# dallison/subspace

Hardware: AMD Instinct MI355X
Metric: GiB/s CRC32 over batched payloads (device-resident); % of HBM3E read peak (higher is better)
Workload: dtype u8

## Files before the change

### subspace_amd/csrc/capi.hip

```cpp
#include <hip/hip_runtime.h>

#include <algorithm>
#include <cstdarg>
#include <cstdio>
#include <cstring>
#include <mutex>
#include <vector>

#include "../../include/subspace_crc.h"
#include "crc_device.h"
#include "crc_math.h"
#include "ctx.h"

namespace subspace_amd {

template <int WG, bool SLOT, bool PROBE>
__global__ void crc32_uniform4k_kernel(const uint8_t*, u64, u64, const u32*, const u32*, u32, u32, u32*, int, u32*,
                                       SlotArgs);

struct TileDesc;
struct TileDesc8;
__global__ void crc32_ragged_count_desc_kernel(const u64*, u32, const u64*, u32, u64, u32, u32, u64*, u32*, u32*,
                                               u64*, u32*, u64, TileDesc8*, u32*, FaultRef);
__global__ void crc32_ragged_count_desc16_kernel(const u64*, u32, const u64*, u32, u64, u32, u32, u64*, u32*, u32*,
                                                 u64*, u32*, u64, TileDesc*, u32*, FaultRef);
__global__ void crc32_ragged_count_scan_kernel(const u64*, u32, const u64*, u32, u64, u32, u32, u64*, u32*, u32*,
                                               u64*, u32*, u32*, FaultRef);
__global__ void tile_segment_scan_kernel(const u32*, u32, u32, u32, const u64*, u64, u32*, u32*);
__global__ void segment_prefix_kernel(u32*, u64, u32, u32, const u64*, u64, u64*, u32*, FaultRef);
__global__ void crc32_ragged_desc_kernel(const u64*, u32, const u64*, u32, const u64*, u64, u64, TileDesc*, u32*,
                                         u64*, u64, u32*, FaultRef);
template <int WG>
__global__ void crc32_ragged_kernel(const uint8_t*, const u64*, u32, const u64*, u32, const u64*, u64,
                                    const TileDesc*, const u32*, const u32*, const u32*, HeadSeeds, u32*, u32*, u32,
                                    u64*, u64, u32*, FaultRef);
__global__ void crc32_ragged_final_kernel(const u64*, const u64*, u32, const u64*, u32, u64, const u32*, const u32*,
                                          u32, u32, u32*, const u32*, u32, u32*, u64*, u64, u32*, FaultRef);
__global__ void crc32_slot_finish_kernel(const u64*, uint8_t*, u64, const u64*, u64, u64, u64, int, int, u32,
                                         const u32*, const u32*, const u32*, u32*, u32*, u32*);
__global__ void slot_payload_offsets_kernel(u64, u64, u64, u64*, const u64*, u64, u64*);
__global__ void uniform_offsets_kernel(u64 stride, u64 length, u64 count, u64* offsets, u64* lengths);
template <int WG>
__global__ void crc32_long_kernel(const uint8_t*, u64, u32, u32, const u32*, const u32*, u32, u32, u32*, u32);
__global__ void crc32_long_final_kernel(const u32*, const u32*, u32, u32, u32, u32, u32*, u64*, u64, u32*);
template <int WG, bool SLOT, bool PROBE, int G>
__global__ void crc32_small_kernel(const u32*, const u32*, SmallArgs);

}

using namespace subspace_amd;

namespace {

thread_local char g_err[512] = "";

int fail(int code, const char* fmt, ...) {
  va_list ap;
  va_start(ap, fmt);
  vsnprintf(g_err, sizeof(g_err), fmt, ap);
  va_end(ap);
  return code;
}
int hip_fail(hipError_t e, const char* what) {
  return fail(SUBSPACE_CRC_EHIP, "%s: %s", what, hipGetErrorString(e));
}
#define HIP_TRY(call)                                   \
  do {                                                  \
    hipError_t e_ = (call);                             \
    if (e_ != hipSuccess) return hip_fail(e_, #call);   \
  } while (0)

constexpr int kRaggedWG = 512;

struct HostRegion {
  uintptr_t host;
  uint64_t bytes;
  uintptr_t dev;
};
std::mutex g_regions_mu;
std::vector<HostRegion> g_regions;

uintptr_t host_alias(uintptr_t p, uint64_t n) {
  for (const auto& r : g_regions)
    if (p >= r.host && p - r.host <= r.bytes && n <= r.bytes - (p - r.host)) return r.dev + (p - r.host);
  return 0;
}
#ifndef SUBSPACE_FINAL_BLOCKS_PER_CU
#define SUBSPACE_FINAL_BLOCKS_PER_CU 2
#endif
constexpr size_t kTileDescBytes = 16;
constexpr u64 ceil_div(u64 a, u64 b) { return (a + b - 1) / b; }

// ... 118 lines not shown
    c->scan_b_words = ceil_div(tile_geom(c, c->desc_capacity).nseg, kScanTile);
    HIP_TRY(hipMalloc(&c->d_scan_state, (1 + c->scan_a_words + c->scan_b_words) * sizeof(u64)));
    HIP_TRY(hipMemset(c->d_scan_state, 0, (1 + c->scan_a_words + c->scan_b_words) * sizeof(u64)));
    HIP_TRY(hipDeviceSynchronize());
    c->scan_dirty = false;
  }
  if (!c->d_overflow) {
    HIP_TRY(hipMalloc(&c->d_overflow, 16));
    HIP_TRY(hipMemset(c->d_overflow, 0, 16));
    HIP_TRY(hipDeviceSynchronize());
  }
  return SUBSPACE_CRC_OK;
}

int scan_state_clean(subspace_crc_ctx* c, hipStream_t st) {
  if (c->scan_dirty) {
    HIP_TRY(hipMemsetAsync(c->d_scan_state, 0, (1 + c->scan_a_words + c->scan_b_words) * sizeof(u64), st));
    c->scan_dirty = false;
  }
  return SUBSPACE_CRC_OK;
}

u64 clamp_capacity(const subspace_crc_ctx* c, u64 cap, u64 count) {
  const u64 lim = std::min<u64>(c->mem_tiles + count + 1, (1ull << 32) - (1ull << 20));
  return std::min(cap, lim);
}

FaultRef new_call_fault(subspace_crc_ctx* c) {
  if (++c->call_gen == 0) c->call_gen = 1;
  return FaultRef{c->d_fault, c->call_gen};
}

int combine_tiles(subspace_crc_ctx* c, const TileGeom& g, const u64* total_ptr, u64 tiles, FaultRef fr,
                  hipStream_t st) {
  const dim3 grid((unsigned)ceil_div(g.nkmax, 64), (unsigned)g.nwb);
  tile_segment_scan_kernel<<<grid, 256, 0, st>>>(c->d_tilecrc, (u32)g.nw, (u32)g.nkmax, (u32)g.nwb, total_ptr, tiles,
                                                  c->d_local, c->d_segx);
  HIP_TRY(hipGetLastError());
  u32* tickets = reinterpret_cast<u32*>(c->d_scan_state);
  segment_prefix_kernel<<<(unsigned)ceil_div(g.nseg, kScanTile), 256, 0, st>>>(
      c->d_segx, g.nseg, (u32)g.nw, (u32)g.nwb, total_ptr, tiles, c->d_scan_state + 1 + c->scan_a_words, tickets + 1,
      fr);
  HIP_TRY(hipGetLastError());
  return SUBSPACE_CRC_OK;
}

int grid_for(subspace_crc_ctx* c, u64 work_units, int waves_per_block) {
  const u64 waves = work_units ? work_units : 1;
  u64 blocks = (waves + waves_per_block - 1) / waves_per_block;
  if (blocks > (u64)c->num_cus) blocks = c->num_cus;
  return (int)(blocks ? blocks : 1);
}

int ragged_run(subspace_crc_ctx* c, const uint8_t* base, u64 cap, const u64* offsets, u32 ostride, const u64* lengths,
               u32 lstride, u64 count, u32 init, u32 final_xor, u32* out, hipStream_t st, u64 arena) {
  int rc = use_workspace(c, st);
  if (rc) return rc;
  cap = clamp_capacity(c, cap, count);
  rc = ensure_ragged_ws(c, count, cap);
  if (rc) return rc;
  const TileGeom g = tile_geom(c, cap);
  const u64 n1 = count + 1;
  rc = scan_state_clean(c, st);
  if (rc) return rc;
  c->scan_dirty = true;
  const FaultRef fr = new_call_fault(c);
  u32* tickets = reinterpret_cast<u32*>(c->d_scan_state);
  const bool fused = c->fused_prep && arena != 0 && arena <= (1ull << kDesc8StartBits) && cap / count <= 64;
  const bool fused16 = c->fused_prep && arena == 0 && cap / count <= 64;
  if (fused) {
    crc32_ragged_count_desc_kernel<<<(unsigned)ceil_div(n1, kCountTile), 1024, 0, st>>>(
        offsets, ostride, lengths, lstride, count, init, final_xor, c->d_tbase, out, c->zero_word, c->d_scan_state + 1,
        reinterpret_cast<u32*>(c->d_scan_state), cap, reinterpret_cast<TileDesc8*>(c->d_desc), c->d_overflow, fr);
    c->zero_word = nullptr;
    HIP_TRY(hipGetLastError());
  } else if (fused16) {
    crc32_ragged_count_desc16_kernel<<<(unsigned)ceil_div(n1, kCountTile), 1024, 0, st>>>(
        offsets, ostride, lengths, lstride, count, init, final_xor, c->d_tbase, out, c->zero_word, c->d_scan_state + 1,
        reinterpret_cast<u32*>(c->d_scan_state), cap, reinterpret_cast<TileDesc*>(c->d_desc), c->d_overflow, fr);
    c->zero_word = nullptr;
    HIP_TRY(hipGetLastError());
  } else {
    crc32_ragged_count_scan_kernel<<<(unsigned)ceil_div(n1, kCountTile), 256, 0, st>>>(
        offsets, ostride, lengths, lstride, count, init, final_xor, c->d_tbase, out, c->zero_word, c->d_scan_state + 1,
        reinterpret_cast<u32*>(c->d_scan_state), c->d_overflow + 1, fr);
    c->zero_word = nullptr;
    HIP_TRY(hipGetLastError());
    const u64 dx = ceil_div(count, 256), waves_x = ceil_div(count, 64);
    const u64 dy = std::max<u64>(1, std::min<u64>({4096, ceil_div(8192, waves_x), cap / count}));
    crc32_ragged_desc_kernel<<<dim3((unsigned)dx, (unsigned)dy), 256, 0, st>>>(
        offsets, ostride, lengths, lstride, c->d_tbase, count, cap, reinterpret_cast<TileDesc*>(c->d_desc),
        c->d_overflow, c->d_scan_state + 1, ceil_div(n1, kCountTile), tickets, fr);
    HIP_TRY(hipGetLastError());
  }
  const int blocks = c->num_cus;
  HeadSeeds seeds;
  seeds.v[0] = init;
  for (int r = 1; r < 16; r++) seeds.v[r] = apply(c->zinv1, seeds.v[r - 1]);
  crc32_ragged_kernel<kRaggedWG><<<blocks, kRaggedWG, ragged_lds_bytes(), st>>>(
      base, offsets, ostride, lengths, lstride, c->d_tbase, count, reinterpret_cast<const TileDesc*>(c->d_desc),
      c->d_overflow, c->d_tab, c->d_rops, seeds, out, c->d_tilecrc, (u32)g.nwb, c->d_scan_state + 1,
      ceil_div(n1, kCountTile), tickets, fr);
  HIP_TRY(hipGetLastError());
  rc = combine_tiles(c, g, c->d_tbase + count, cap, fr, st);
  if (rc) return rc;
  const u64 fb = SUBSPACE_FINAL_BLOCKS_PER_CU ? std::min<u64>(ceil_div(count, 1024), (u64)SUBSPACE_FINAL_BLOCKS_PER_CU * c->num_cus)
                                              : ceil_div(count, 1024);
  crc32_ragged_final_kernel<<<(unsigned)fb, 1024, 0, st>>>(
      c->d_tbase, offsets, ostride, lengths, lstride, count, c->d_local, c->d_segx, (u32)g.nw, (u32)g.nwb,
      c->d_overflow, c->d_rops, final_xor, out, c->d_scan_state + 1 + c->scan_a_words, ceil_div(g.nseg, kScanTile),
      tickets + 1, fr);
  HIP_TRY(hipGetLastError());
  c->scan_dirty = false;
  return SUBSPACE_CRC_OK;
}

bool small_fits(u64 max_len, bool aligned16) { return max_len <= (aligned16 ? kSmallMaxExt : kSmallMaxExt - 15); }

u32 small_lanes(u64 max_ext) {
  if (max_ext == 0) return 32;
  u32 g = 1;
  while (g < 32 && 128ull * g < max_ext) g <<= 1;
  return g;
}

struct SmallSlot {
  const u64* prefixes;
  u32 pstride;
  u64 pdelta;
  u64 max_len;
  u32 mode;
  int32_t checksum_size, metadata_size;
  u32 *status, *crc_out, *error_count;
};
int small_run(subspace_crc_ctx* c, const uint8_t* base, const u64* offsets, u32 ostride, const u64* lengths,
              u32 lstride, u64 count, u32 init, u32 final_xor, u32* out, hipStream_t st,
              const SmallSlot* slot = nullptr, u32 g = 32, u64 ustride = 0, u64 ulen = 0) {
  SmallArgs a{};
  a.ustride = ustride;
  a.ulen = ulen;
  a.base = base;
  a.offsets = offsets;
  a.ostride = ostride;
  a.lengths = lengths;
  a.lstride = lstride;
  a.count = count;
  a.init = init;
  a.final_xor = final_xor;
  a.out = out;
  a.rops = c->d_rops;
  a.pow2 = c->d_pow2;
  a.probe = c->dev.probe;
  const bool probe = c->dev.probe && c->dev.small_slot;
  if (probe) g = 32;
  const u64 tiles = ceil_div(count, 64ull / g);
  const u64 per_wave = slot && g == 32 ? kRp2MaxTilesPerWave : kSmallRingTiles;
// ... 33 lines not shown
#undef SMALL_CASE
    }
  }
  HIP_TRY(hipGetLastError());
  return SUBSPACE_CRC_OK;
}

bool small_slot_fused(int32_t checksum_size, int32_t metadata_size) {
  return (u32)checksum_size <= kSlotFusedMaxMeta && (u32)metadata_size <= kSlotFusedMaxMeta;
}

int ensure_slot_ws(subspace_crc_ctx* c, u64 count) {
  if (count <= c->s_capacity) return SUBSPACE_CRC_OK;
  (void)hipFree(c->d_crc0);
  (void)hipFree(c->d_soff);
  (void)hipFree(c->d_slen);
  c->d_crc0 = nullptr;
  c->d_soff = nullptr;
  c->d_slen = nullptr;
  c->s_capacity = 0;
  HIP_TRY(hipMalloc(&c->d_crc0, count * sizeof(u32)));
  HIP_TRY(hipMalloc(&c->d_soff, count * sizeof(u64)));
  HIP_TRY(hipMalloc(&c->d_slen, count * sizeof(u64)));
  c->s_capacity = count;
  return SUBSPACE_CRC_OK;
}

int check_slot_args(int32_t checksum_size, int32_t metadata_size, uint32_t mode) {
  if (mode != SUBSPACE_CRC_SLOT_CALCULATE && mode != SUBSPACE_CRC_SLOT_VERIFY)
    return fail(SUBSPACE_CRC_EINVAL, "unknown slot mode %u", mode);
  if (checksum_size < 4) return fail(SUBSPACE_CRC_EINVAL, "checksum_size %d < 4", checksum_size);
  if (metadata_size < 0) return fail(SUBSPACE_CRC_EINVAL, "metadata_size %d < 0", metadata_size);
  return SUBSPACE_CRC_OK;
}

void want_zeroed(subspace_crc_ctx* c, u32* err) { c->zero_word = err; }
bool was_zeroed(subspace_crc_ctx* c, u32* err) {
  const bool z = err && c->zero_word == nullptr;
  c->zero_word = nullptr;
  return z;
}

int slot_finish(subspace_crc_ctx* c, const u64* slots, uint8_t* buf, u64 stride, const u64* sizes, u64 usize,
                u64 count, u64 max_len, int32_t cs, int32_t ms, u32 mode, u32* status, u32* err, hipStream_t st,
                u32* crc_out = nullptr, bool err_zeroed = false) {
  if (err && !err_zeroed) HIP_TRY(hipMemsetAsync(err, 0, sizeof(u32), st));
  crc32_slot_finish_kernel<<<(unsigned)((count + 255) / 256), 256, 0, st>>>(
      slots, buf, stride, sizes, usize, count, max_len, cs, ms, mode, c->d_crc0, c->d_tab, c->d_pow2, status, err,
      crc_out);
  HIP_TRY(hipGetLastError());
  return SUBSPACE_CRC_OK;
}

}

extern "C" {

int subspace_crc_version(void) { return 100; }

const char* subspace_crc_last_error(void) { return g_err; }

int subspace_crc_ctx_create(int device, subspace_crc_ctx** out) {
  return subspace_crc_ctx_create_poly(device, SUBSPACE_CRC_POLY_IEEE, out);
}

int subspace_crc_ctx_create_poly(int device, uint32_t poly, subspace_crc_ctx** out) {
  g_err[0] = 0;
  if (!out) return fail(SUBSPACE_CRC_EINVAL, "out is null");
  *out = nullptr;
  if (!(poly & 0x80000000u)) return fail(SUBSPACE_CRC_EINVAL, "polynomial 0x%08x has no x^0 term", poly);
  int ndev = 0;
  if (hipGetDeviceCount(&ndev) != hipSuccess || ndev == 0)
    return fail(SUBSPACE_CRC_ENODEV, "no HIP device available");
  if (device < 0 || device >= ndev) return fail(SUBSPACE_CRC_EINVAL, "device %d out of range [0,%d)", device, ndev);
  hipDeviceProp_t prop;
  HIP_TRY(hipGetDeviceProperties(&prop, device));
  if (std::strncmp(prop.gcnArchName, "gfx950", 6) != 0)
    return fail(SUBSPACE_CRC_ENODEV, "device %d is %s, this library is built for gfx950", device, prop.gcnArchName);
  HIP_TRY(hipSetDevice(device));

  auto* c = new subspace_crc_ctx();
  c->layout_bytes = (uint32_t)sizeof(subspace_crc_ctx);
  c->device = device;
  c->num_cus = prop.multiProcessorCount;
  c->mem_tiles = (u64)prop.totalGlobalMem / 8192;
  c->poly = poly;
  c->host_tab = make_tables(poly);
  c->zinv1 = inverse(z_one(c->host_tab));

  std::vector<u32> tab(1024), pow2(64 * 128, 0u), laneops(kSmallLaneOpSlots * 128, 0u), rops(kRagOpWords, 0u);
  for (int k = 0; k < 4; k++)
    for (int b = 0; b < 256; b++) tab[k * 256 + b] = c->host_tab.t[k][b];

  {
    Mat32 z = z_one(c->host_tab);
    for (int k = 0; k < 64; k++, z = mul(z, z)) nibble_tables(z, &pow2[(size_t)k * 128]);
  }

  for (int sl = 0; sl < 32; sl++) {
    u32 nt[128];
    nibble_tables(z_bytes(c->host_tab, 128ull * sl), nt);
    for (int k = 0; k < 8; k++)
      for (int n = 0; n < 16; n++) laneops[((size_t)k * 16 + n) * 32 + sl] = nt[k * 16 + n];
  }
  std::copy(laneops.begin(), laneops.begin() + kLaneOpWords, rops.begin());
  nibble_tables(z_bytes(c->host_tab, 4096), &laneops[128 * kUniSlotOpZ4096]);
// ... 206 lines not shown
        c->d_scan_state + 1 + c->scan_a_words, ceil_div(g.nseg, kScanTile), reinterpret_cast<u32*>(c->d_scan_state) + 1);
    HIP_TRY(hipGetLastError());
    c->scan_dirty = false;
    return SUBSPACE_CRC_OK;
  }
  const bool aligned = (stride % 16) == 0 && ((uintptr_t)dev_base % 16) == 0;
  if (small_fits(length, aligned) && c->small_path && count > 1)
    return small_run(c, static_cast<const uint8_t*>(dev_base), nullptr, 0, nullptr, 0, count, init, final_xor,
                     dev_out, st, nullptr, small_lanes(length + (aligned ? 0 : 15)), stride, length);
  int rc = use_workspace(c, st);
  if (rc) return rc;
  if (count > c->u_capacity) {
    (void)hipFree(c->d_uoff);
    (void)hipFree(c->d_ulen);
    c->d_uoff = c->d_ulen = nullptr;
    c->u_capacity = 0;
    HIP_TRY(hipMalloc(&c->d_uoff, count * sizeof(u64)));
    HIP_TRY(hipMalloc(&c->d_ulen, count * sizeof(u64)));
    c->u_capacity = count;
  }
  uniform_offsets_kernel<<<(unsigned)((count + 255) / 256), 256, 0, st>>>(stride, length, count, c->d_uoff,
                                                                           c->d_ulen);
  HIP_TRY(hipGetLastError());
  const u64 arena = stride * (count - 1) + length;
  return subspace_crc32_batch(c, dev_base, arena, c->d_uoff, c->d_ulen, count, init, flags, dev_out, stream);
}

int subspace_crc32_slots(subspace_crc_ctx* c, const subspace_crc_slot* dev_slots, uint64_t count,
                         uint64_t max_message_size, int32_t checksum_size, int32_t metadata_size, uint32_t mode,
                         uint32_t* dev_status, uint32_t* dev_error_count, void* stream) {
  g_err[0] = 0;
  if (!c) return fail(SUBSPACE_CRC_EINVAL, "ctx is null");
  CallScope scope(c);
  int rc = check_slot_args(checksum_size, metadata_size, mode);
  if (rc) return rc;
  hipStream_t st = (hipStream_t)stream;
  if (count == 0) {
    if (dev_error_count) HIP_TRY(hipMemsetAsync(dev_error_count, 0, sizeof(u32), st));
    return SUBSPACE_CRC_OK;
  }
  if (!dev_slots) return fail(SUBSPACE_CRC_EINVAL, "null device pointer");
  if (count >= (1ull << 32)) return fail(SUBSPACE_CRC_EINVAL, "count %llu exceeds 2^32-1", (unsigned long long)count);
  HIP_TRY(hipSetDevice(c->device));
  const u64* rec = reinterpret_cast<const u64*>(dev_slots);
  const bool small = max_message_size <= kSmallMaxExt && c->small_path;
  if (small && small_slot_fused(checksum_size, metadata_size)) {
    const SmallSlot ss{rec, 3, 0, ~0ull, mode, checksum_size, metadata_size, dev_status, nullptr, dev_error_count};
    return small_run(c, nullptr, rec + 1, 3, rec + 2, 3, count, 0u, 0u, nullptr, st, &ss, small_lanes(max_message_size));
  }
  rc = use_workspace(c, st);
  if (rc) return rc;
  rc = ensure_slot_ws(c, count);
  if (rc) return rc;
  want_zeroed(c, dev_error_count);
  if (small) {
    rc = small_run(c, nullptr, rec + 1, 3, rec + 2, 3, count, 0u, 0u, c->d_crc0, st, nullptr,
                   small_lanes(max_message_size));
  } else {
    const u64 cap = count * ((max_message_size + 15 + 8191) / 8192) + 1;
    rc = ragged_run(c, nullptr, cap, rec + 1, 3, rec + 2, 3, count, 0u, 0u, c->d_crc0, st, 0);
  }
  const bool zeroed = was_zeroed(c, dev_error_count);
  if (rc) return rc;
  return slot_finish(c, rec, nullptr, 0, nullptr, 0, count, ~0ull, checksum_size, metadata_size, mode, dev_status,
                     dev_error_count, st, nullptr, zeroed);
}

}

namespace {

int slots_strided_impl(subspace_crc_ctx* c, void* dev_buffer, uint64_t slot_stride, uint64_t count,
                       uint64_t message_size, const uint64_t* dev_message_sizes, int32_t checksum_size,
                       int32_t metadata_size, uint32_t mode, uint32_t* dev_status, uint32_t* dev_error_count,
                       u32* dev_crc_out, hipStream_t st) {
  int rc = check_slot_args(checksum_size, metadata_size, mode);
  if (rc) return rc;
  if (count == 0) {
    if (dev_error_count) HIP_TRY(hipMemsetAsync(dev_error_count, 0, sizeof(u32), st));
    return SUBSPACE_CRC_OK;
  }
  if (!dev_buffer) return fail(SUBSPACE_CRC_EINVAL, "null device pointer");
  if (((uintptr_t)dev_buffer % 8) || (slot_stride % 8))
    return fail(SUBSPACE_CRC_EINVAL, "prefixes must be 8-B aligned (buffer %p, stride %llu)", dev_buffer,
                (unsigned long long)slot_stride);
  if (count >= (1ull << 32)) return fail(SUBSPACE_CRC_EINVAL, "count %llu exceeds 2^32-1", (unsigned long long)count);
  const u64 prefix_size = ((u64)(48 + checksum_size + metadata_size) + 63) & ~63ull;
  if (!dev_message_sizes && slot_stride < prefix_size + message_size && count > 1)
    return fail(SUBSPACE_CRC_EINVAL, "slot_stride %llu < prefix %llu + message %llu",
                (unsigned long long)slot_stride, (unsigned long long)prefix_size, (unsigned long long)message_size);
  if (dev_message_sizes && slot_stride < prefix_size && count > 1)
    return fail(SUBSPACE_CRC_EINVAL, "slot_stride %llu < prefix %llu", (unsigned long long)slot_stride,
                (unsigned long long)prefix_size);
  HIP_TRY(hipSetDevice(c->device));
  auto* buf = static_cast<uint8_t*>(dev_buffer);
  if (!dev_message_sizes && message_size == 4096 && (u32)metadata_size <= kSlotFusedMaxMeta && slot_stride % 16 == 0 &&
      ((uintptr_t)(buf + prefix_size) % 16) == 0 && c->fused_slots) {
    const u64 tiles = (count + 1) / 2;
    const u64 blocks = std::max<u64>(grid_for(c, tiles, 512 / 64), ceil_div(tiles, 8ull * kSlotRingRounds));
    SlotArgs sa{prefix_size, mode, dev_status, dev_crc_out, dev_error_count,
                c->d_slot_counter + kCountWords * (c->slot_counter_next++ % kSlotCounters), c->dev.probe, c->d_fault,
                (u32)checksum_size, (u32)metadata_size};
    if (c->dev.probe && c->dev.uniform)
      HIP_TRY(c->dev.uniform(true, (unsigned)blocks, st, buf + prefix_size, slot_stride, count, c->d_tab, c->d_laneops,
                             0u, 0xFFFFFFFFu, nullptr, nullptr, sa));
    else
      crc32_uniform4k_kernel<512, true, false><<<(unsigned)blocks, 512, uniform_slot_lds_bytes(8), st>>>(
          buf + prefix_size, slot_stride, count, c->d_tab, c->d_laneops, 0u, 0xFFFFFFFFu, nullptr, 0, nullptr, sa);
    HIP_TRY(hipGetLastError());
    return SUBSPACE_CRC_OK;
  }
  rc = use_workspace(c, st);
  if (rc) return rc;
  rc = ensure_slot_ws(c, count);
  if (rc) return rc;
  want_zeroed(c, dev_error_count);
  if (dev_message_sizes) {
    const u64 area = count > 1 ? slot_stride - prefix_size : ~0ull;
    slot_payload_offsets_kernel<<<(unsigned)((count + 255) / 256), 256, 0, st>>>(
        slot_stride, prefix_size, count, c->d_soff, dev_message_sizes, area, c->d_slen);
    HIP_TRY(hipGetLastError());
    const bool aligned = slot_stride % 16 == 0 && ((uintptr_t)(buf + prefix_size) % 16) == 0;
    if (count > 1 && small_fits(slot_stride - prefix_size, aligned) && c->small_path) {
      if (small_slot_fused(checksum_size, metadata_size)) {
        was_zeroed(c, dev_error_count);
        const SmallSlot ss{c->d_soff, 1, prefix_size, slot_stride - prefix_size, mode, checksum_size, metadata_size,
                           dev_status, dev_crc_out, dev_error_count};
        return small_run(c, buf, c->d_soff, 1, dev_message_sizes, 1, count, 0u, 0u, nullptr, st, &ss,
                         small_lanes(slot_stride - prefix_size + (aligned ? 0 : 15)));
      }
      rc = small_run(c, buf, c->d_soff, 1, c->d_slen, 1, count, 0u, 0u, c->d_crc0, st, nullptr,
                     small_lanes(slot_stride - prefix_size + (aligned ? 0 : 15)));
    } else {
      const u64 cap = (slot_stride * count + 15 * count) / 8192 + count + 1;
      rc = ragged_run(c, buf, cap, c->d_soff, 1, c->d_slen, 1, count, 0u, 0u, c->d_crc0, st,
                      slot_stride * count);
    }
  } else {
    rc = subspace_crc32_batch_uniform(c, buf + prefix_size, slot_stride, message_size, count, 0u, 0u, c->d_crc0,
                                      st);
  }
  const bool zeroed = was_zeroed(c, dev_error_count);
  if (rc) return rc;
  const u64 max_len = dev_message_sizes && count > 1 ? slot_stride - prefix_size : ~0ull;
  return slot_finish(c, nullptr, buf, slot_stride, dev_message_sizes, message_size, count, max_len, checksum_size,
                     metadata_size, mode, dev_status, dev_error_count, st, dev_crc_out, zeroed);
}

}

extern "C" {

int subspace_crc32_slots_strided(subspace_crc_ctx* c, void* dev_buffer, uint64_t slot_stride, uint64_t count,
                                 uint64_t message_size, const uint64_t* dev_message_sizes, int32_t checksum_size,
                                 int32_t metadata_size, uint32_t mode, uint32_t* dev_status,
                                 uint32_t* dev_error_count, void* stream) {
  g_err[0] = 0;
  if (!c) return fail(SUBSPACE_CRC_EINVAL, "ctx is null");
  CallScope scope(c);
  return slots_strided_impl(c, dev_buffer, slot_stride, count, message_size, dev_message_sizes, checksum_size,
                            metadata_size, mode, dev_status, dev_error_count, nullptr, (hipStream_t)stream);
}

int subspace_crc_host_register(void* ptr, uint64_t bytes) {
  g_err[0] = 0;
  if (!ptr || !bytes) return fail(SUBSPACE_CRC_EINVAL, "null pointer or zero size");
  HIP_TRY(hipHostRegister(ptr, bytes, hipHostRegisterMapped | hipHostRegisterPortable));
  void* dev = nullptr;
  hipError_t e = hipHostGetDevicePointer(&dev, ptr, 0);
  if (e != hipSuccess) {
    (void)hipHostUnregister(ptr);
    return hip_fail(e, "hipHostGetDevicePointer");
  }
  std::lock_guard<std::mutex> lock(g_regions_mu);
  g_regions.push_back({reinterpret_cast<uintptr_t>(ptr), bytes, reinterpret_cast<uintptr_t>(dev)});
  return SUBSPACE_CRC_OK;
}

int subspace_crc_host_unregister(void* ptr) {
  g_err[0] = 0;
  if (!ptr) return fail(SUBSPACE_CRC_EINVAL, "null pointer");
  {
    std::lock_guard<std::mutex> lock(g_regions_mu);
    for (size_t i = 0; i < g_regions.size(); i++)
      if (g_regions[i].host == reinterpret_cast<uintptr_t>(ptr)) {
        g_regions.erase(g_regions.begin() + (long)i);
        break;
// ... 225 lines not shown
```

### subspace_amd/csrc/crc_combine.hip

```cpp
#include "crc_desc.h"

namespace subspace_amd {

constexpr int kScanThreads = 256;
constexpr int kScanItems = (int)(kScanTile / kScanThreads);
static_assert(kScanTile % kScanThreads == 0, "segment-prefix scan: whole items per thread");
constexpr int kCountItems = (int)(kCountTile / kScanThreads);
static_assert(kCountTile % kScanThreads == 0, "tile-count scan: whole items per thread");
constexpr u64 kFlagAggregate = 1, kFlagInclusive = 2;

struct SumOp {
  using T = u64;
  static __device__ __forceinline__ T identity() { return 0; }
  static __device__ __forceinline__ T op(T a, T b) { return a + b; }
  static __device__ __forceinline__ u64 pack(u64 flag, T v) { return (flag << 62) | v; }
  static __device__ __forceinline__ u64 flag(u64 s) { return s >> 62; }
  static __device__ __forceinline__ T value(u64 s) { return s & ((1ull << 62) - 1); }
};

struct XorOp {
  using T = u32;
  static __device__ __forceinline__ T identity() { return 0; }
  static __device__ __forceinline__ T op(T a, T b) { return a ^ b; }
  static __device__ __forceinline__ u64 pack(u64 flag, T v) { return (flag << 32) | v; }
// ... 116 lines not shown
  __shared__ u64 sx[kCountTile];
  bool stale;
  const u64 tile = scan_ticket(ticket, fault, &stale, true);
  if (stale) return;
  const u64 base = tile * kCountTile;
  const int tid = threadIdx.x;
#pragma unroll
  for (int j = 0; j < kCountItems; j++) {
    const u64 i = base + (u64)(j * kScanThreads + tid);
    u64 nt = 0;
    if (i < count) {
      const u64 so = offsets[i * ostride];
      nt = msg_tiles(so, lengths[i * lstride]);
      out[i] = nt == 0 ? init ^ final_xor : 0u;
      if (nt && ((((so & ~(u64)15) + ((nt - 1) << 13)) >> kDesc8StartBits) | ((nt - 1) >> kDesc8AfterBits)))
        *wide = 1u;
    } else if (i == count && zero_word) {
      *zero_word = 0u;
    }
    sx[j * kScanThreads + tid] = nt;
  }
  __syncthreads();
  u64 x[kCountItems];
#pragma unroll
  for (int j = 0; j < kCountItems; j++) x[j] = sx[tid * kCountItems + j];
  scan_tile_lookback<SumOp, kCountItems>(x, tile, status, fault);
#pragma unroll
  for (int j = 0; j < kCountItems; j++) sx[tid * kCountItems + j] = x[j];
  __syncthreads();
#pragma unroll
  for (int j = 0; j < kCountItems; j++) {
    const u64 i = base + (u64)(j * kScanThreads + tid);
    if (i <= count) tile_base[i] = sx[j * kScanThreads + tid];
  }
}

constexpr int kFusedThreads = 1024;
constexpr int kFusedItems = (int)(kCountTile / kFusedThreads);
static_assert(kCountTile % kFusedThreads == 0, "fused scan: whole items per thread");
template <bool WIDE>
__device__ __forceinline__ void count_desc_body(const u64* __restrict__ offsets, u32 ostride,
                                                const u64* __restrict__ lengths, u32 lstride, u64 count, u32 init,
                                                u32 final_xor, u64* __restrict__ tile_base, u32* __restrict__ out,
                                                u32* __restrict__ zero_word, u64* __restrict__ status,
                                                u32* __restrict__ ticket, u64 capacity, void* __restrict__ desc,
                                                u32* __restrict__ overflow, FaultRef fault) {
  __shared__ u64 sx[kCountTile];
  __shared__ u32 sw[WIDE ? 1 : kFusedThreads / 64][kDesc8WaveWords][64];
  bool stale;
  const u64 tile = scan_ticket(ticket, fault, &stale, true);
  if (stale) return;
  const u64 base = tile * kCountTile;
  const int tid = threadIdx.x;
  if (WIDE && tid == 0) overflow[1] = 1u;
  u64 so[kFusedItems], L[kFusedItems], nt[kFusedItems];
  bool bad = false;
#pragma unroll
  for (int j = 0; j < kFusedItems; j++) {
    const u64 i = base + (u64)(j * kFusedThreads + tid);
    so[j] = L[j] = nt[j] = 0;
    if (i < count) {
      so[j] = offsets[i * ostride];
      L[j] = lengths[i * lstride];
      nt[j] = msg_tiles(so[j], L[j]);
      out[i] = nt[j] == 0 ? init ^ final_xor : 0u;
      if (!WIDE && nt[j] &&
          ((((so[j] & ~(u64)15) + ((nt[j] - 1) << 13)) >> kDesc8StartBits) | ((nt[j] - 1) >> kDesc8AfterBits)))
        bad = true;
    } else if (i == count && zero_word) {
      *zero_word = 0u;
    }
    sx[j * kFusedThreads + tid] = nt[j];
  }
  if (bad) overflow[2] = 1u;
  __syncthreads();
  u64 x[kFusedItems];
#pragma unroll
  for (int j = 0; j < kFusedItems; j++) x[j] = sx[tid * kFusedItems + j];
  scan_tile_lookback<SumOp, kFusedItems, kFusedThreads>(x, tile, status, fault);
#pragma unroll
  for (int j = 0; j < kFusedItems; j++) sx[tid * kFusedItems + j] = x[j];
  __syncthreads();
#pragma unroll
  for (int j = 0; j < kFusedItems; j++) {
    const u64 i = base + (u64)(j * kFusedThreads + tid);
    const u64 tb = sx[j * kFusedThreads + tid];
    if (i <= count) tile_base[i] = tb;
    if (i == count) overflow[0] = tb > capacity ? 1u : 0u;
    if constexpr (WIDE)
      descw_wave(static_cast<TileDesc*>(desc), capacity, tb, nt[j], so[j], L[j]);
    else
      desc8_wave(static_cast<TileDesc8*>(desc), capacity, tb, nt[j], so[j], L[j], 0u, 64u, sw[tid >> 6], true);
  }
}

__global__ __launch_bounds__(kFusedThreads) void crc32_ragged_count_desc_kernel(
    const u64* __restrict__ offsets, u32 ostride, const u64* __restrict__ lengths, u32 lstride, u64 count, u32 init,
    u32 final_xor, u64* __restrict__ tile_base, u32* __restrict__ out, u32* __restrict__ zero_word,
    u64* __restrict__ status, u32* __restrict__ ticket, u64 capacity, TileDesc8* __restrict__ desc8,
    u32* __restrict__ overflow, FaultRef fault) {
  count_desc_body<false>(offsets, ostride, lengths, lstride, count, init, final_xor, tile_base, out, zero_word, status,
                         ticket, capacity, desc8, overflow, fault);
}

__global__ __launch_bounds__(kFusedThreads) void crc32_ragged_count_desc16_kernel(
    const u64* __restrict__ offsets, u32 ostride, const u64* __restrict__ lengths, u32 lstride, u64 count, u32 init,
    u32 final_xor, u64* __restrict__ tile_base, u32* __restrict__ out, u32* __restrict__ zero_word,
// ... 92 lines not shown
```

### subspace_amd/csrc/crc_slots.hip

```cpp
#include "crc_device.h"

namespace subspace_amd {

constexpr int kSlotWG = 256;
constexpr u32 kHasChecksum = 4u;

__device__ __forceinline__ u32 tab_step4(const u32* __restrict__ t, u32 x) {
  return t[768 + (x & 0xFFu)] ^ t[512 + ((x >> 8) & 0xFFu)] ^ t[256 + ((x >> 16) & 0xFFu)] ^ t[x >> 24];
}
__device__ __forceinline__ u32 tab_step1(const u32* __restrict__ t, u32 crc, u32 b) {
  return (crc >> 8) ^ t[(crc ^ b) & 0xFFu];
}

__device__ u32 crc_bytes(const u32* __restrict__ t, u32 crc, const uint8_t* p, u64 n) {
  while (n && ((uintptr_t)p & 3u)) {
    crc = tab_step1(t, crc, *p++);
    n--;
  }
  const u32* q = reinterpret_cast<const u32*>(p);
  for (; n >= 4; n -= 4) crc = tab_step4(t, crc ^ *q++);
  p = reinterpret_cast<const uint8_t*>(q);
  while (n--) crc = tab_step1(t, crc, *p++);
  return crc;
}

__global__ __launch_bounds__(kSlotWG) void crc32_slot_finish_kernel(
    const u64* __restrict__ slots, uint8_t* __restrict__ buf, u64 stride, const u64* __restrict__ sizes, u64 usize,
    u64 count, u64 max_len, int checksum_size, int metadata_size, u32 mode, const u32* __restrict__ crc0,
    const u32* __restrict__ gtab, const u32* __restrict__ gpow2, u32* __restrict__ status,
    u32* __restrict__ error_count, u32* __restrict__ crc_out) {
  __shared__ u32 t[1024];
  constexpr int kPowLds = 16;
  __shared__ u32 pw2[kPowLds * 128];
  for (int i = threadIdx.x; i < 1024; i += kSlotWG) t[i] = gtab[i];
  for (int i = threadIdx.x; i < kPowLds * 128; i += kSlotWG) pw2[i] = gpow2[i];
  __syncthreads();
  const u64 i = (u64)blockIdx.x * kSlotWG + threadIdx.x;
  if (i >= count) return;
  uint8_t* prefix = slots ? reinterpret_cast<uint8_t*>(slots[3 * i]) : buf + i * stride;
  const u64 len = slots ? slots[3 * i + 2] : (sizes ? sizes[i] : usize);
  u32* pw = reinterpret_cast<u32*>(prefix);
  if (len > max_len) {
    if (status) status[i] = 4u;
    return;
  }

  u32 w[12];
#pragma unroll
  for (int k = 1; k < 12; k++) w[k] = pw[k];
  const bool calc = mode == 0u;
  const bool has = (w[8] & kHasChecksum) != 0u;
  if (calc && !has) {
    w[8] |= kHasChecksum;
    pw[8] = w[8];
  }
  if (!calc && !has) {
    if (status) status[i] = 2u;
    return;
  }
  u32 h = 0xFFFFFFFFu;
#pragma unroll
  for (int k = 1; k < 12; k++) h = tab_step4(t, h ^ w[k]);
  if (metadata_size > 0) h = crc_bytes(t, h, prefix + 48 + checksum_size, (u64)metadata_size);
  u32 zh = h;
  {
    u64 n = len;
    for (int k = 0; n; k++, n >>= 1) {
      if (!(n & 1u)) continue;
      const u32* op = k < kPowLds ? pw2 + 128 * k : gpow2 + 128 * k;
      u32 r = 0;
#pragma unroll
      for (int j = 0; j < 8; j++) r ^= op[16 * j + ((zh >> (4 * j)) & 15u)];
      zh = r;
    }
  }
  const u32 crc = ~(zh ^ crc0[i]);
  if (calc) {
    pw[12] = crc;
    if (status) status[i] = 0u;
    if (crc_out) crc_out[i] = crc;
  } else {
    const bool ok = pw[12] == crc;
    if (status) status[i] = ok ? 0u : 1u;
    if (!ok && error_count) atomicAdd(error_count, 1u);
  }
}

__global__ void slot_payload_offsets_kernel(u64 stride, u64 prefix_size, u64 count, u64* __restrict__ offsets,
                                            const u64* __restrict__ sizes, u64 max_len, u64* __restrict__ clamped) {
  const u64 i = (u64)blockIdx.x * blockDim.x + threadIdx.x;
  if (i >= count) return;
  offsets[i] = i * stride + prefix_size;
  const u64 L = sizes[i];
  clamped[i] = L > max_len ? 0 : L;
}

}
```

### subspace_amd/csrc/ctx.h

```cpp
#pragma once
#include <hip/hip_runtime.h>

#include <mutex>

#include "../../include/subspace_crc.h"
#include "crc_device.h"
#include "crc_math.h"

namespace subspace_amd {

struct DevHooks {
  u64* probe = nullptr;
  hipError_t (*uniform)(bool slot, unsigned blocks, hipStream_t st, const uint8_t* base, u64 stride, u64 count,
                        const u32* tab, const u32* ops, u32 init, u32 final_xor, u32* out, u32* zero_word,
                        SlotArgs sa) = nullptr;
  hipError_t (*small_slot)(unsigned blocks, size_t lds, hipStream_t st, const u32* tab, const u32* ops,
                           const SmallArgs& a) = nullptr;
};

constexpr uint32_t kCtxMagic = 0x43524353u;

}

struct subspace_crc_ctx {
// ... 4 lines not shown
  int num_cus = 256;
  subspace_amd::u32* d_tab = nullptr;
  subspace_amd::u32* d_rops = nullptr;
  subspace_amd::u32* d_pow2 = nullptr;
  subspace_amd::u32* d_laneops = nullptr;
  subspace_amd::Tables host_tab;
  subspace_amd::Mat32 zinv1;
  subspace_amd::u64* d_tbase = nullptr;
  subspace_amd::u64 ws_messages = 0;
  uint8_t* d_desc = nullptr;
  subspace_amd::u32* d_tilecrc = nullptr;
  subspace_amd::u32* d_local = nullptr;
  subspace_amd::u32* d_segx = nullptr;
  subspace_amd::u64 desc_capacity = 0;
  subspace_amd::u64* d_scan_state = nullptr;
  subspace_amd::u64 scan_a_words = 0, scan_b_words = 0;
  bool scan_dirty = false;
  subspace_amd::u64 mem_tiles = 0;
  subspace_amd::u32* d_overflow = nullptr;
  bool fused_prep = true;
  int uniform_blocks = 0;
  int uniform_order = 0;
  bool long_path = true;
  subspace_amd::u32* zero_word = nullptr;
  subspace_amd::u64* d_uoff = nullptr;
  subspace_amd::u64* d_ulen = nullptr;
  subspace_amd::u64 u_capacity = 0;
  hipStream_t hcompute = nullptr;
  struct HostStage {
    hipStream_t stream = nullptr;
    hipEvent_t copied = nullptr;
    hipEvent_t done = nullptr;
    uint8_t* dbuf = nullptr;
    subspace_amd::u64* dsizes = nullptr;
    subspace_amd::u32* dres = nullptr;
    subspace_amd::u32* derr = nullptr;
    subspace_amd::u32* hres = nullptr;
    subspace_amd::u32* herr = nullptr;
  } hstage[2];
  subspace_amd::u64 h_bytes = 0, h_slots = 0;
  subspace_crc_slot* l_hrec = nullptr;
  subspace_crc_slot* l_drec = nullptr;
  subspace_amd::u32* l_dstatus = nullptr;
  subspace_amd::u32* l_hstatus = nullptr;
  subspace_amd::u64 l_capacity = 0;
  subspace_amd::u32* d_crc0 = nullptr;
  subspace_amd::u64* d_soff = nullptr;
  subspace_amd::u64* d_slen = nullptr;
  subspace_amd::u64 s_capacity = 0;
  subspace_amd::u64* d_slot_counter = nullptr;
  subspace_amd::u32 slot_counter_next = 0;
  bool fused_slots = true;
  bool small_path = true;
  subspace_amd::DevHooks dev;
  subspace_amd::u32* d_fault = nullptr;
  subspace_amd::u32 call_gen = 0;
  std::recursive_mutex mu;
  int depth = 0;
  hipEvent_t ws_done = nullptr;
  hipStream_t ws_stream = nullptr;
  bool ws_recorded = false;
  bool ws_waited = false;
  hipStream_t ws_call_stream = nullptr;
};
```

### subspace_amd/csrc/devtools.hip

```cpp
#define SUBSPACE_DEV_TU 1
#include "crc_small.hip"
#include "crc_uniform.hip"
#include "ctx.h"

#include <algorithm>
#include <cstring>

namespace subspace_amd {
template __global__ void crc32_small_kernel<512, true, true, 32>(const u32*, const u32*, SmallArgs);
template __global__ void crc32_uniform4k_kernel<512, false, true>(const uint8_t*, u64, u64, const u32*, const u32*, u32,
                                                                  u32, u32*, int, u32*, SlotArgs);
template __global__ void crc32_uniform4k_kernel<512, true, true>(const uint8_t*, u64, u64, const u32*, const u32*, u32,
                                                                 u32, u32*, int, u32*, SlotArgs);
template __global__ void crc32_uniform4k_kernel<512, false, false>(const uint8_t*, u64, u64, const u32*, const u32*,
                                                                   u32, u32, u32*, int, u32*, SlotArgs);
}

using namespace subspace_amd;

namespace {

bool ctx_ok(const subspace_crc_ctx* c) {
  return c && c->magic == kCtxMagic && c->layout_bytes == (uint32_t)sizeof(subspace_crc_ctx);
}
// ... 9 lines not shown
                         SlotArgs sa) {
  if (slot)
    crc32_uniform4k_kernel<512, true, true><<<blocks, 512, uniform_slot_lds_bytes(8), st>>>(
        base, stride, count, tab, ops, init, final_xor, out, 0, zero_word, sa);
  else
    crc32_uniform4k_kernel<512, false, true><<<blocks, 512, uniform_lds_bytes(8), st>>>(
        base, stride, count, tab, ops, init, final_xor, out, 0, zero_word, sa);
  return hipGetLastError();
}

hipError_t small_slot_probe(unsigned blocks, size_t lds, hipStream_t st, const u32* tab, const u32* ops,
                            const SmallArgs& a) {
  crc32_small_kernel<512, true, true, 32><<<blocks, 512, lds, st>>>(tab, ops, a);
  return hipGetLastError();
}

hipError_t set_lds_attributes() {
  static hipError_t e = [] {
    hipError_t r = hipFuncSetAttribute((const void*)crc32_uniform4k_kernel<512, false, true>,
                                       hipFuncAttributeMaxDynamicSharedMemorySize, (int)uniform_lds_bytes(8));
    if (r == hipSuccess)
      r = hipFuncSetAttribute((const void*)crc32_uniform4k_kernel<512, true, true>,
                              hipFuncAttributeMaxDynamicSharedMemorySize, (int)uniform_slot_lds_bytes(8));
    if (r == hipSuccess)
      r = hipFuncSetAttribute((const void*)crc32_uniform4k_kernel<512, false, false>,
                              hipFuncAttributeMaxDynamicSharedMemorySize, (int)uniform_lds_bytes(8));
    if (r == hipSuccess)
      r = hipFuncSetAttribute((const void*)crc32_small_kernel<512, true, true, 32>,
                              hipFuncAttributeMaxDynamicSharedMemorySize, (int)small_lds_bytes() + 16);
    return r;
  }();
  return e;
}

}

extern "C" {

int subspace_crc_testutil_set(subspace_crc_ctx* c, const char* key, int value) {
  if (!ctx_ok(c) || !key) return SUBSPACE_CRC_EINVAL;
  std::lock_guard<std::recursive_mutex> lk(c->mu);
  if (!std::strcmp(key, "stale_ticket")) {
    if (!c->d_scan_state) return SUBSPACE_CRC_EINVAL;
    const u32 v = (u32)value;
    if (hipSetDevice(c->device) != hipSuccess || hipDeviceSynchronize() != hipSuccess ||
        hipMemcpy(c->d_scan_state, &v, sizeof(u32), hipMemcpyHostToDevice) != hipSuccess)
      return SUBSPACE_CRC_EHIP;
    return SUBSPACE_CRC_OK;
  }
  bool* knob = !std::strcmp(key, "long_path")     ? &c->long_path
               : !std::strcmp(key, "fused_slots") ? &c->fused_slots
               : !std::strcmp(key, "fused_prep")  ? &c->fused_prep
               : !std::strcmp(key, "small_path")  ? &c->small_path
                                                  : nullptr;
  if (!knob) return SUBSPACE_CRC_EINVAL;
  *knob = value != 0;
  return SUBSPACE_CRC_OK;
}

int subspace_crc_testutil_tune(subspace_crc_ctx* c, int uniform_wg, int uniform_blocks, int uniform_order) {
  if (!ctx_ok(c) || uniform_wg != 512 || uniform_order < 0 || uniform_order > 3 || uniform_blocks < 0)
    return SUBSPACE_CRC_EINVAL;
  std::lock_guard<std::recursive_mutex> lk(c->mu);
  c->uniform_blocks = uniform_blocks;
  c->uniform_order = uniform_order;
  return SUBSPACE_CRC_OK;
}

int subspace_crc_testutil_probe(subspace_crc_ctx* c, void* dev_words) {
  if (!ctx_ok(c)) return SUBSPACE_CRC_EINVAL;
  std::lock_guard<std::recursive_mutex> lk(c->mu);
  if (dev_words) {
    if (hipSetDevice(c->device) != hipSuccess || set_lds_attributes() != hipSuccess) return SUBSPACE_CRC_EHIP;
    c->dev.uniform = uniform_probe;
    c->dev.small_slot = small_slot_probe;
  }
  c->dev.probe = static_cast<u64*>(dev_words);
  return SUBSPACE_CRC_OK;
}

uint64_t subspace_crc_testutil_probe_waves(subspace_crc_ctx* c, uint64_t count) {
  if (!ctx_ok(c)) return 0;
  const u64 tiles = (count + 1) / 2;
  return std::max<u64>((u64)blocks_for(c, tiles), (tiles + 8ull * kRp2MaxTilesPerWave - 1) / (8ull * kRp2MaxTilesPerWave)) * 8u;
}

int subspace_crc_testutil_uniform_alias(subspace_crc_ctx* c, const void* dev_base, uint64_t count, uint32_t* dev_out,
                                        void* stream) {
  if (!ctx_ok(c) || !dev_base || !dev_out || count == 0 || ((uintptr_t)dev_base % 16)) return SUBSPACE_CRC_EINVAL;
  std::lock_guard<std::recursive_mutex> lk(c->mu);
  if (hipSetDevice(c->device) != hipSuccess || set_lds_attributes() != hipSuccess) return SUBSPACE_CRC_EHIP;
  const u64 tiles = (count + 1) / 2;
  crc32_uniform4k_kernel<512, false, false><<<blocks_for(c, tiles), 512, uniform_lds_bytes(8), (hipStream_t)stream>>>(
      static_cast<const uint8_t*>(dev_base), 0, count, c->d_tab, c->d_laneops, 0u, 0u, dev_out, 0, nullptr, SlotArgs{});
  return hipGetLastError() == hipSuccess ? SUBSPACE_CRC_OK : SUBSPACE_CRC_EHIP;
}

int subspace_crc_testutil_fault_words(subspace_crc_ctx* c, uint32_t* host_words, void* stream) {
  if (!ctx_ok(c) || !host_words) return SUBSPACE_CRC_EINVAL;
  std::lock_guard<std::recursive_mutex> lk(c->mu);
  if (hipSetDevice(c->device) != hipSuccess ||
      hipMemcpyAsync(host_words, c->d_fault, 2 * sizeof(u32), hipMemcpyDeviceToHost, (hipStream_t)stream) != hipSuccess ||
      hipStreamSynchronize((hipStream_t)stream) != hipSuccess)
    return SUBSPACE_CRC_EHIP;
  return SUBSPACE_CRC_OK;
}

// ... 4 lines not shown
```

Baseline: 5642.

## Fuse ragged tile combine and final pass into slot finish kernel

For slot-based ragged CRC with bounded message sizes, the tile-combine scan, segment prefix and ragged final kernels are skipped. A new slot_combine_finish kernel XORs each message's tile CRCs directly, undoes the padding shift with nibble inverse operators held in LDS, and writes the checksum or verifies it in the same pass. This removes several kernel launches and their intermediate global traffic, at the cost of a serial per-message loop over tiles that is limited to a small tile count.

```diff
diff --git a/subspace_amd/csrc/capi.hip b/subspace_amd/csrc/capi.hip
--- a/subspace_amd/csrc/capi.hip
+++ b/subspace_amd/csrc/capi.hip
@@ -38,6 +38,11 @@
                                           u32, u32, u32*, const u32*, u32, u32*, u64*, u64, u32*, FaultRef);
 __global__ void crc32_slot_finish_kernel(const u64*, uint8_t*, u64, const u64*, u64, u64, u64, int, int, u32,
                                          const u32*, const u32*, const u32*, u32*, u32*, u32*);
+template <bool LIST>
+__global__ void crc32_slot_combine_finish_kernel(const u64*, uint8_t*, u64, const u64*, u64, u64, int, int, u32,
+                                                 const u64*, const u64*, u32, const u64*, u32, const u32*, u32, u32,
+                                                 u32*, const u32*, const u32*, const u32*, const u32*, u32*, u32*,
+                                                 u32*, FaultRef);
 __global__ void slot_payload_offsets_kernel(u64, u64, u64, u64*, const u64*, u64, u64*);
 __global__ void uniform_offsets_kernel(u64 stride, u64 length, u64 count, u64* offsets, u64* lengths);
 template <int WG>
@@ -262,8 +267,14 @@
   return (int)(blocks ? blocks : 1);
 }
 
+struct RaggedTiles {
+  TileGeom g;
+  FaultRef fr;
+};
+
 int ragged_run(subspace_crc_ctx* c, const uint8_t* base, u64 cap, const u64* offsets, u32 ostride, const u64* lengths,
-               u32 lstride, u64 count, u32 init, u32 final_xor, u32* out, hipStream_t st, u64 arena) {
+               u32 lstride, u64 count, u32 init, u32 final_xor, u32* out, hipStream_t st, u64 arena,
+               RaggedTiles* tiles_only = nullptr) {
   int rc = use_workspace(c, st);
   if (rc) return rc;
   cap = clamp_capacity(c, cap, count);
@@ -312,6 +323,11 @@
       c->d_overflow, c->d_tab, c->d_rops, seeds, out, c->d_tilecrc, (u32)g.nwb, c->d_scan_state + 1,
       ceil_div(n1, kCountTile), tickets, fr);
   HIP_TRY(hipGetLastError());
+  if (tiles_only) {
+    tiles_only->g = g;
+    tiles_only->fr = fr;
+    return SUBSPACE_CRC_OK;
+  }
   rc = combine_tiles(c, g, c->d_tbase + count, cap, fr, st);
   if (rc) return rc;
   const u64 fb = SUBSPACE_FINAL_BLOCKS_PER_CU ? std::min<u64>(ceil_div(count, 1024), (u64)SUBSPACE_FINAL_BLOCKS_PER_CU * c->num_cus)
@@ -451,6 +467,38 @@
   return SUBSPACE_CRC_OK;
 }
 
+constexpr u64 kSlotCombineMaxTiles = 8;
+constexpr int kSlotCombineWG = 256;
+bool slot_combine_fits(const subspace_crc_ctx* c, u64 bound) {
+  return c->slot_combine && bound <= kSlotCombineMaxTiles * 8192 - 15;
+}
+
+int ragged_slot_combine(subspace_crc_ctx* c, const uint8_t* base, u64 cap, const u64* offsets, u32 ostride,
+                        const u64* lengths, u32 lstride, u64 arena, const u64* slots, uint8_t* buf, u64 stride,
+                        const u64* sizes, u64 count, u64 max_len, int32_t cs, int32_t ms, u32 mode, u32* status,
+                        u32* err, u32* crc_out, hipStream_t st) {
+  want_zeroed(c, err);
+  RaggedTiles rt;
+  const int rc = ragged_run(c, base, cap, offsets, ostride, lengths, lstride, count, 0u, 0u, c->d_crc0, st, arena, &rt);
+  const bool zeroed = was_zeroed(c, err);
+  if (rc) return rc;
+  if (err && !zeroed) HIP_TRY(hipMemsetAsync(err, 0, sizeof(u32), st));
+  const unsigned grid = (unsigned)ceil_div(count, kSlotCombineWG);
+  if (slots)
+    crc32_slot_combine_finish_kernel<true><<<grid, kSlotCombineWG, 0, st>>>(
+        slots, buf, stride, sizes, count, max_len, cs, ms, mode, c->d_tbase, offsets, ostride, lengths, lstride,
+        c->d_tilecrc, (u32)rt.g.nw, (u32)rt.g.nwb, c->d_overflow, c->d_crc0, c->d_tab, c->d_pow2, c->d_rops, status,
+        err, crc_out, rt.fr);
+  else
+    crc32_slot_combine_finish_kernel<false><<<grid, kSlotCombineWG, 0, st>>>(
+        slots, buf, stride, sizes, count, max_len, cs, ms, mode, c->d_tbase, offsets, ostride, lengths, lstride,
+        c->d_tilecrc, (u32)rt.g.nw, (u32)rt.g.nwb, c->d_overflow, c->d_crc0, c->d_tab, c->d_pow2, c->d_rops, status,
+        err, crc_out, rt.fr);
+  HIP_TRY(hipGetLastError());
+  c->scan_dirty = false;
+  return SUBSPACE_CRC_OK;
+}
+
 }
 
 extern "C" {
@@ -763,12 +811,15 @@
   if (rc) return rc;
   rc = ensure_slot_ws(c, count);
   if (rc) return rc;
+  const u64 cap = count * ((max_message_size + 15 + 8191) / 8192) + 1;
+  if (!small && slot_combine_fits(c, max_message_size))
+    return ragged_slot_combine(c, nullptr, cap, rec + 1, 3, rec + 2, 3, 0, rec, nullptr, 0, nullptr, count, ~0ull,
+                               checksum_size, metadata_size, mode, dev_status, dev_error_count, nullptr, st);
   want_zeroed(c, dev_error_count);
   if (small) {
     rc = small_run(c, nullptr, rec + 1, 3, rec + 2, 3, count, 0u, 0u, c->d_crc0, st, nullptr,
                    small_lanes(max_message_size));
   } else {
-    const u64 cap = count * ((max_message_size + 15 + 8191) / 8192) + 1;
     rc = ragged_run(c, nullptr, cap, rec + 1, 3, rec + 2, 3, count, 0u, 0u, c->d_crc0, st, 0);
   }
   const bool zeroed = was_zeroed(c, dev_error_count);
@@ -844,6 +895,12 @@
                      small_lanes(slot_stride - prefix_size + (aligned ? 0 : 15)));
     } else {
       const u64 cap = (slot_stride * count + 15 * count) / 8192 + count + 1;
+      if (count > 1 && slot_combine_fits(c, slot_stride - prefix_size)) {
+        was_zeroed(c, dev_error_count);
+        return ragged_slot_combine(c, buf, cap, c->d_soff, 1, c->d_slen, 1, slot_stride * count, nullptr, buf,
+                                   slot_stride, dev_message_sizes, count, area, checksum_size, metadata_size, mode,
+                                   dev_status, dev_error_count, dev_crc_out, st);
+      }
       rc = ragged_run(c, buf, cap, c->d_soff, 1, c->d_slen, 1, count, 0u, 0u, c->d_crc0, st,
                       slot_stride * count);
     }
diff --git a/subspace_amd/csrc/crc_combine.hip b/subspace_amd/csrc/crc_combine.hip
--- a/subspace_amd/csrc/crc_combine.hip
+++ b/subspace_amd/csrc/crc_combine.hip
@@ -192,7 +192,7 @@
   if (stale) return;
   const u64 base = tile * kCountTile;
   const int tid = threadIdx.x;
-  if (WIDE && tid == 0) overflow[1] = 1u;
+  if (tid == 0) overflow[1] = WIDE ? 1u : 0u;
   u64 so[kFusedItems], L[kFusedItems], nt[kFusedItems];
   bool bad = false;
 #pragma unroll
diff --git a/subspace_amd/csrc/crc_slots.hip b/subspace_amd/csrc/crc_slots.hip
--- a/subspace_amd/csrc/crc_slots.hip
+++ b/subspace_amd/csrc/crc_slots.hip
@@ -24,22 +24,15 @@
   return crc;
 }
 
-__global__ __launch_bounds__(kSlotWG) void crc32_slot_finish_kernel(
-    const u64* __restrict__ slots, uint8_t* __restrict__ buf, u64 stride, const u64* __restrict__ sizes, u64 usize,
-    u64 count, u64 max_len, int checksum_size, int metadata_size, u32 mode, const u32* __restrict__ crc0,
-    const u32* __restrict__ gtab, const u32* __restrict__ gpow2, u32* __restrict__ status,
-    u32* __restrict__ error_count, u32* __restrict__ crc_out) {
-  __shared__ u32 t[1024];
-  constexpr int kPowLds = 16;
-  __shared__ u32 pw2[kPowLds * 128];
-  for (int i = threadIdx.x; i < 1024; i += kSlotWG) t[i] = gtab[i];
-  for (int i = threadIdx.x; i < kPowLds * 128; i += kSlotWG) pw2[i] = gpow2[i];
-  __syncthreads();
-  const u64 i = (u64)blockIdx.x * kSlotWG + threadIdx.x;
-  if (i >= count) return;
-  uint8_t* prefix = slots ? reinterpret_cast<uint8_t*>(slots[3 * i]) : buf + i * stride;
-  const u64 len = slots ? slots[3 * i + 2] : (sizes ? sizes[i] : usize);
-  u32* pw = reinterpret_cast<u32*>(prefix);
+constexpr int kPowLds = 16;
+template <class Payload>
+__device__ __forceinline__ void slot_finish_one(const u32* __restrict__ t, const u32* __restrict__ pw2,
+                                                const u32* __restrict__ gpow2, u64 i, uint8_t* prefix, u64 len,
+                                                u64 max_len, int checksum_size, int metadata_size, u32 mode,
+                                                u32* __restrict__ status, u32* __restrict__ error_count,
+                                                u32* __restrict__ crc_out, Payload payload) {
+  typedef __attribute__((address_space(1))) u32 global_u32_t;
+  global_u32_t* pw = reinterpret_cast<global_u32_t*>(reinterpret_cast<uintptr_t>(prefix));
   if (len > max_len) {
     if (status) status[i] = 4u;
     return;
@@ -48,6 +41,7 @@
   u32 w[12];
 #pragma unroll
   for (int k = 1; k < 12; k++) w[k] = pw[k];
+  const u32 crc0 = payload();
   const bool calc = mode == 0u;
   const bool has = (w[8] & kHasChecksum) != 0u;
   if (calc && !has) {
@@ -74,7 +68,7 @@
       zh = r;
     }
   }
-  const u32 crc = ~(zh ^ crc0[i]);
+  const u32 crc = ~(zh ^ crc0);
   if (calc) {
     pw[12] = crc;
     if (status) status[i] = 0u;
@@ -86,6 +80,131 @@
   }
 }
 
+__global__ __launch_bounds__(kSlotWG) void crc32_slot_finish_kernel(
+    const u64* __restrict__ slots, uint8_t* __restrict__ buf, u64 stride, const u64* __restrict__ sizes, u64 usize,
+    u64 count, u64 max_len, int checksum_size, int metadata_size, u32 mode, const u32* __restrict__ crc0,
+    const u32* __restrict__ gtab, const u32* __restrict__ gpow2, u32* __restrict__ status,
+    u32* __restrict__ error_count, u32* __restrict__ crc_out) {
+  __shared__ u32 t[1024];
+  __shared__ u32 pw2[kPowLds * 128];
+  for (int i = threadIdx.x; i < 1024; i += kSlotWG) t[i] = gtab[i];
+  for (int i = threadIdx.x; i < kPowLds * 128; i += kSlotWG) pw2[i] = gpow2[i];
+  __syncthreads();
+  const u64 i = (u64)blockIdx.x * kSlotWG + threadIdx.x;
+  if (i >= count) return;
+  uint8_t* prefix = slots ? reinterpret_cast<uint8_t*>(slots[3 * i]) : buf + i * stride;
+  const u64 len = slots ? slots[3 * i + 2] : (sizes ? sizes[i] : usize);
+  slot_finish_one(t, pw2, gpow2, i, prefix, len, max_len, checksum_size, metadata_size, mode, status, error_count,
+                  crc_out, [&] { return crc0[i]; });
+}
+
+constexpr int kSlotCombineUnroll = 8;
+constexpr int kSlotCombineWG = 256;
+__device__ __forceinline__ void pin_loaded(u64& v) {
+  u32 lo = (u32)v, hi = (u32)(v >> 32);
+  asm volatile("" : "+v"(lo), "+v"(hi));
+  v = ((u64)hi << 32) | lo;
+}
+__device__ __forceinline__ void pin_loaded(u32& v) { asm volatile("" : "+v"(v)); }
+
+template <bool LIST>
+__global__ __launch_bounds__(kSlotCombineWG) void crc32_slot_combine_finish_kernel(
+    const u64* __restrict__ slots, uint8_t* __restrict__ buf, u64 stride, const u64* __restrict__ sizes, u64 count,
+    u64 max_len, int checksum_size, int metadata_size, u32 mode, const u64* __restrict__ tile_base,
+    const u64* __restrict__ offsets, u32 ostride, const u64* __restrict__ lengths, u32 lstride,
+    const u32* __restrict__ tilecrc, u32 nw, u32 nwb, u32* __restrict__ overflow, const u32* __restrict__ crc0,
+    const u32* __restrict__ gtab, const u32* __restrict__ gpow2, const u32* __restrict__ gops,
+    u32* __restrict__ status, u32* __restrict__ error_count, u32* __restrict__ crc_out, FaultRef fault) {
+  constexpr int kT = 0, kPw2 = 1024, kInv = kPw2 + kPowLds * 128, kInvZ = kInv + kNumNibInvOps * 128;
+  constexpr int kWords = kInvZ + 128, kIters = (kWords + kSlotCombineWG - 1) / kSlotCombineWG;
+  __shared__ u32 lds[kWords];
+  const u32 *t = lds + kT, *pw2 = lds + kPw2, *inv = lds + kInv;
+  if (blockIdx.x == 0 && threadIdx.x == 0) overflow[1] = overflow[2] = 0u;
+  if (scan_faulted(fault)) return;
+  u32 sv[kIters];
+#pragma unroll
+  for (int i = 0; i < kIters; i++) {
+    const int j = min((int)threadIdx.x + i * kSlotCombineWG, kWords - 1);
+    const u32* src = j < kPw2 ? gtab + j : j < kInv ? gpow2 + (j - kPw2)
+                   : j < kInvZ ? gops + kRagNibInvOps + (j - kInv) : gops + kRagInvOps + 128 * 12 + (j - kInvZ);
+    sv[i] = *src;
+  }
+  const bool ovf = overflow[0] != 0u;
+  const u64 m = (u64)blockIdx.x * kSlotCombineWG + threadIdx.x;
+  const u64 mc = m < count ? m : count - 1;
+  u64 pfx = LIST ? slots[3 * mc] : 0;
+  u64 len = LIST ? slots[3 * mc + 2] : sizes[mc];
+  u64 t0 = tile_base[mc], t1 = tile_base[mc + 1];
+  u64 sm = LIST ? slots[3 * mc + 1] : offsets[mc * ostride];
+  u64 Lm = LIST ? len : lengths[mc * lstride];
+  u32 c0 = crc0[mc];
+#pragma unroll
+  for (int i = 0; i < kIters; i++) {
+    const int j = (int)threadIdx.x + i * kSlotCombineWG;
+    if (j < kWords) lds[j] = sv[i];
+  }
+  __syncthreads();
+  if (m >= count) return;
+  pin_loaded(pfx);
+  pin_loaded(len);
+  pin_loaded(t0);
+  pin_loaded(t1);
+  pin_loaded(sm);
+  pin_loaded(Lm);
+  pin_loaded(c0);
+  uint8_t* prefix = LIST ? reinterpret_cast<uint8_t*>(pfx) : buf + m * stride;
+  slot_finish_one(t, pw2, gpow2, m, prefix, len, max_len, checksum_size, metadata_size, mode, status, error_count,
+                  crc_out, [&]() -> u32 {
+    if (t1 == t0) return c0;
+    u32 k = (u32)t0 / nw, w = (u32)t0 - k * nw;
+    const u64 n = ovf ? 0 : t1 - t0;
+    u32 x[kSlotCombineUnroll];
+#pragma unroll
+    for (int j = 0; j < kSlotCombineUnroll; j++) {
+      const bool in = (u64)j < n;
+      x[j] = tilecrc[in ? tilecrc_index(w, k, nwb) : 0];
+      if (++w == nw) {
+        w = 0;
+        k++;
+      }
+    }
+    u32 v = ovf ? c0 : 0u;
+#pragma unroll
+    for (int j = 0; j < kSlotCombineUnroll; j++) v ^= (u64)j < n ? x[j] : 0u;
+    for (u64 j = kSlotCombineUnroll; j < n; j++) {
+      v ^= tilecrc[tilecrc_index(w, k, nwb)];
+      if (++w == nw) {
+        w = 0;
+        k++;
+      }
+    }
+    auto undo = [&](u32 slot, u32 y) {
+      const u32* op = inv + 128 * slot;
+      u32 r = op[y & 15u];
+#pragma unroll
+      for (int q = 1; q < 8; q++) r ^= op[16 * q + ((y >> (4 * q)) & 15u)];
+      return r;
+    };
+    const u32 pad = (u32)(0 - (Lm + (sm & 15))) & 8191u;
+#pragma unroll
+    for (u32 q = 0; q < 3; q++) {
+      const u32 d = (pad >> (4 * q)) & 15u;
+      if (d) v = undo(15 * q + d - 1, v);
+    }
+    if (pad & 0x1000u) v = undo(kNumNibInvOps, v);
+    return v;
+  });
+}
+
+template __global__ void crc32_slot_combine_finish_kernel<true>(const u64*, uint8_t*, u64, const u64*, u64, u64, int,
+                                                                int, u32, const u64*, const u64*, u32, const u64*, u32,
+                                                                const u32*, u32, u32, u32*, const u32*, const u32*,
+                                                                const u32*, const u32*, u32*, u32*, u32*, FaultRef);
+template __global__ void crc32_slot_combine_finish_kernel<false>(const u64*, uint8_t*, u64, const u64*, u64, u64, int,
+                                                                 int, u32, const u64*, const u64*, u32, const u64*, u32,
+                                                                 const u32*, u32, u32, u32*, const u32*, const u32*,
+                                                                 const u32*, const u32*, u32*, u32*, u32*, FaultRef);
+
 __global__ void slot_payload_offsets_kernel(u64 stride, u64 prefix_size, u64 count, u64* __restrict__ offsets,
                                             const u64* __restrict__ sizes, u64 max_len, u64* __restrict__ clamped) {
   const u64 i = (u64)blockIdx.x * blockDim.x + threadIdx.x;
diff --git a/subspace_amd/csrc/ctx.h b/subspace_amd/csrc/ctx.h
--- a/subspace_amd/csrc/ctx.h
+++ b/subspace_amd/csrc/ctx.h
@@ -80,6 +80,7 @@
   subspace_amd::u32 slot_counter_next = 0;
   bool fused_slots = true;
   bool small_path = true;
+  bool slot_combine = true;
   subspace_amd::DevHooks dev;
   subspace_amd::u32* d_fault = nullptr;
   subspace_amd::u32 call_gen = 0;
diff --git a/subspace_amd/csrc/devtools.hip b/subspace_amd/csrc/devtools.hip
--- a/subspace_amd/csrc/devtools.hip
+++ b/subspace_amd/csrc/devtools.hip
@@ -85,7 +85,8 @@
                : !std::strcmp(key, "fused_slots") ? &c->fused_slots
                : !std::strcmp(key, "fused_prep")  ? &c->fused_prep
                : !std::strcmp(key, "small_path")  ? &c->small_path
-                                                  : nullptr;
+               : !std::strcmp(key, "slot_combine") ? &c->slot_combine
+                                                   : nullptr;
   if (!knob) return SUBSPACE_CRC_EINVAL;
   *knob = value != 0;
   return SUBSPACE_CRC_OK;
```

After: 5567. 0.987x the previous value.
